# qfall/tools

Measured on AMD Instinct MI355X. Metric: preimages/sec (whole node) + HBM-BW% for samp_p, n=512 q~2^30 batch=4096, higher is better.
Workload: dtype f64+int64

## Files before the change

include/psf_mi355x.h:

```cpp
#ifndef PSF_MI355X_H
#define PSF_MI355X_H
#include <stddef.h>
#include <stdint.h>

#ifdef __cplusplus
extern "C" {
#endif

typedef int psf_status;
enum {
  PSF_OK = 0,
  PSF_ERR_PARAM = 1,
  PSF_ERR_NOT_PD = 2,
  PSF_ERR_DOMAIN = 3,
  PSF_ERR_MODULUS = 4,
  PSF_ERR_NO_SOLUTION = 5,
  PSF_ERR_NO_KEY = 6,
  PSF_ERR_HIP = 7,
  PSF_ERR_UNSUPPORTED = 8,
  PSF_ERR_SAMPLER = 9
};

const char* psf_status_string(psf_status);
psf_status psf_device_info(int device, char* name, size_t name_len, int* compute_units);
// ... 162 lines not shown

psf_status psfp_samp_p_dev(psfp_handle*, uint64_t seed, uint64_t first_index, size_t B,
                           const uint64_t* d_u, int64_t* d_e, void* stream);
psf_status psfp_samp_p_dev_many(psfp_handle*, size_t count, const uint64_t* seeds, const uint64_t* first_indices, size_t B,
                                const uint64_t* d_u, int64_t* d_e, void* stream);
psf_status psfp_samp_d_dev(psfp_handle*, uint64_t seed, uint64_t first_index, size_t B, int64_t* d_e, void* stream);
psf_status psfp_f_a_dev(psfp_handle*, size_t B, const int64_t* d_e, uint64_t* d_u, uint8_t* d_ok, void* stream);
psf_status psfp_last_status(psfp_handle*);
psf_status psfp_uniform_targets_dev(psfp_handle*, uint64_t seed, uint64_t first_index, size_t B, uint64_t* d_u, void* stream);
psf_status psf_narrow_rows_dev(const int64_t* d_src, int32_t* d_dst, size_t count, int* d_overflow, int device, void* stream);

psf_status psfp_samp_p_stages(psfp_handle*, uint64_t seed, uint64_t first_index, size_t B, const uint64_t* u,
                              double* d, double* x, int64_t* p, uint64_t* v, int64_t* z, int64_t* e);
psf_status psfp_enable_timing(psfp_handle*, int on);
psf_status psfp_get_timing(psfp_handle*, char* names, size_t names_len, double* ms, size_t* count);
enum {
  PSFP_PLAN_ONE_LAUNCH = 0,
  PSFP_PLAN_PRODUCT,
  PSFP_PLAN_RT, PSFP_PLAN_NB, PSFP_PLAN_NCG,
  PSFP_PLAN_BC,
  PSFP_PLAN_COMPACT,
  PSFP_PLAN_GR, PSFP_PLAN_GC,
  PSFP_PLAN_TAIL,
  PSFP_PLAN_ROUND,
  PSFP_PLAN_SYN_FORM,
  PSFP_PLAN_SYN_SPLITS, PSFP_PLAN_SYN_FOLD128, PSFP_PLAN_SYN_POW2, PSFP_PLAN_SYN_WAVE_COMBINE,
  PSFP_PLAN_GADGET,
  PSFP_PLAN_K32,
  PSFP_PLAN_GQ_P,
  PSFP_PLAN_RECOMBINE,
  PSFP_PLAN_NBF,
  PSFP_PLAN_RC_BIG,
  PSFP_PLAN_RSPLITS,
  PSFP_PLAN_FIELDS
};
enum { PSFP_PRODUCT_TASKS = 0, PSFP_PRODUCT_TILES64 = 1, PSFP_PRODUCT_TILES32 = 2, PSFP_PRODUCT_TILES96 = 3, PSFP_PRODUCT_BIG = 4 };
enum { PSFP_ROUND_TAB = 0, PSFP_ROUND_TAB_ROW = 1, PSFP_ROUND_LEAN = 2, PSFP_ROUND_WAVE = 3 };
enum { PSFP_ZQ_SMALL = 0, PSFP_ZQ_SMALL32 = 1, PSFP_ZQ_MFMA = 2 };
enum { PSFP_GADGET_WAVE = 0, PSFP_GADGET_ROW = 1, PSFP_GADGET_QUAD = 2, PSFP_GADGET_QUEUE = 3, PSFP_GADGET_LOCKSTEP = 4 };
enum { PSFP_RECOMBINE_SMALL = 0, PSFP_RECOMBINE_SMALL2 = 1, PSFP_RECOMBINE_WG = 2, PSFP_RECOMBINE_TILES = 3 };
psf_status psfp_query_plan(const psfp_handle*, size_t B, int* fields, size_t count);
psf_status psfp_get_last_plan(const psfp_handle*, int* fields, size_t count);

typedef struct psfgpv_handle psfgpv_handle;
typedef struct {
  psf_gadget_params gp;
  double s;
  int32_t device;
  uint32_t flags;
} psfgpv_params;

psf_status psfgpv_create(const psfgpv_params* params, psfgpv_handle** out);
void       psfgpv_destroy(psfgpv_handle*);
size_t     psfgpv_m(const psfgpv_handle*);
psf_status psfgpv_trap_gen(psfgpv_handle*, uint64_t seed);
psf_status psfgpv_load_key(psfgpv_handle*, const uint64_t* A, const int32_t* basis_t, const double* gso_t);
psf_status psfgpv_export_key(const psfgpv_handle*, uint64_t* A, int8_t* R, int32_t* basis_t, double* gso_t);
psf_status psfgpv_samp_d(psfgpv_handle*, uint64_t seed, uint64_t first_index, size_t B, int64_t* e);
psf_status psfgpv_samp_p(psfgpv_handle*, uint64_t seed, uint64_t first_index, size_t B, const uint64_t* u, int64_t* e);
psf_status psfgpv_samp_p_dev(psfgpv_handle*, uint64_t seed, uint64_t first_index, size_t B, const uint64_t* d_u, int64_t* d_e, void* stream);
psf_status psfgpv_samp_p_dev_many(psfgpv_handle*, size_t count, const uint64_t* seeds, const uint64_t* first_indices, size_t B,
                                  const uint64_t* d_u, int64_t* d_e, void* stream);
psf_status psfgpv_samp_p_async(psfgpv_handle*, uint64_t seed, uint64_t first_index, size_t B, const uint64_t* u, int64_t* e);
psf_status psfgpv_wait(psfgpv_handle*);
uint64_t   psfgpv_async_next_ticket(const psfgpv_handle*);
psf_status psfgpv_wait_ticket(psfgpv_handle*, uint64_t ticket);
// ... 48 lines not shown
```

tools_amd/csrc/psfp.hip:

```cpp
#include <hip/hip_runtime.h>
#include <cmath>
#include <cstdio>
#include <cstdlib>
#include <cstring>
#include <chrono>
#include <string>
#include <thread>
#include <atomic>
#include <mutex>
#include <functional>
#include <vector>
#include "psf_hip_util.hpp"
#include "psf_host.hpp"
#include "psf_kernels.hpp"
#include "psf_stream_kernels.hpp"
#include "psf_gpv_kernels.hpp"
#include "psf_np_kernels.hpp"
#include "psf_chol_kernels.hpp"
#include "psf_gemm_kernels.hpp"
#include "psf_hostpipe.hpp"
#include "psf_ntt_api.hpp"

struct KeygenClock {
  bool on; const char* what; std::chrono::steady_clock::time_point t0, last;
  explicit KeygenClock(const char* w) : on(psf_exp_env("PSF_KEYGEN_TIMING") != nullptr), what(w) { if (on) { hipDeviceSynchronize(); t0 = last = std::chrono::steady_clock::now(); } }
  void mark(const char* phase) {
    if (!on) return;
    hipDeviceSynchronize();
    const auto now = std::chrono::steady_clock::now();
    std::fprintf(stderr, "[keygen %s] %-28s %8.2f ms (at %8.2f)\n", what, phase, std::chrono::duration<double, std::milli>(now - last).count(), std::chrono::duration<double, std::milli>(now - t0).count());
    last = now;
  }
};

#define PSFP_FLAG_NO_PERTURB 1u

using namespace psf;

static inline unsigned grid_for(size_t total, unsigned block = 256, unsigned cap = 256 * 16) {
  size_t g = (total + block - 1) / block;
  if (g < 1) g = 1;
  return (unsigned)(g > cap ? cap : g);
}
#define PSFP_QUIESCE(h) do { const psf_status rw__ = psfp_wait(h); if (rw__ != PSF_OK) return rw__; } while (0)

struct TimingSlot { std::string name; Event e0, e1; };

// ... 17 lines not shown
  bool wide;
  bool has_key = false;
  NormBound dom = {{0, 0, 0}};
  bool has_pub = false;
  bool has_R = false;
  DevArr<uint64_t> dA;
  DevArr<int8_t> dR;
  size_t ldr = 0;
  DevArr<double> dLt;
  size_t M_pad = 0, nbi = 0, nkb = 0;
  bool structured = false;
  size_t mL = 0, nbiL = 0;
  DevArr<int8_t> dR8;
  bool r8_valid = false;
  bool r8_pending = false;
  Event evR8; hipStream_t r8_stream = nullptr;
  DevArr<uint32_t> dR2, dA32; DevArr<int> dR2bad; PinArr<int> hR2bad; Event evSmall;
  DevArr<uint32_t> dA32T;
  DevArr<uint64_t> dPartF;
  int small_state = 0;
  double g_const = 0, h_const = 0;
  DevArr<int32_t> dRng;
  DevArr<int32_t> dSk; DevArr<double> dGso, dNorm2; DevArr<SampleZParams> dSz;
  DevArr<uint64_t> dGvec;
  DevArr<int8_t> dA8; int NA = 0; size_t n_pad = 0, K_pad = 0;
  ZqConsts zc;
  std::vector<int64_t> hSk; std::vector<double> hGso;
  SampleZParams szR, szSR;
  DevArr<uint32_t> dSzTab; uint32_t szF = 0;
  size_t ld = 0, mb_pad = 0;
  DevArr<int> dFail;
  int zq_split_cap = 1;
  bool gadget_queue = true;
  HostPipe hp;
  uint32_t normals_ncf = 0;
  hipStream_t last_stream = nullptr;
  Stream side; Event evSide;
  bool timing = false;
  std::vector<TimingSlot> slots;
  double multi_launched_ms = -1.0, multi_done_ms = -1.0;
  int last_plan[PSFP_PLAN_FIELDS] = {0}; bool has_last_plan = false;
};

static void ensure_small_copies(psfp_handle* h, hipStream_t st) {
  if ((h->prm.flags & PSFP_FLAG_NO_PERTURB) || h->small_state >= 2) return;
  if (h->small_state == 1) {
    if (hipEventQuery(h->evSmall) == hipSuccess) h->small_state = *h->hR2bad ? 3 : 2;
    return;
  }
  const size_t ng = h->ldr / 16;
  if (!h->dR2) {
    if (h->dR2.alloc(h->mb * ng) != hipSuccess || h->dR2bad.alloc(1) != hipSuccess ||
        h->hR2bad.alloc(1) != hipSuccess || hipEventCreateWithFlags(h->evSmall.put(), hipEventDisableTiming) != hipSuccess) { h->small_state = 4; return; }
    if (h->q <= (1ull << 32) && h->dA32.alloc(h->n * h->m) != hipSuccess) { h->small_state = 4; return; }
    if (h->q <= (1ull << 32) && h->n % 8 == 0 && h->dA32T.alloc(h->n * h->m) != hipSuccess) (void)hipGetLastError();
  }
  hipMemsetAsync(h->dR2bad, 0, sizeof(int), st);
  hipLaunchKernelGGL(k_pack_R2, dim3(grid_for(h->mb * ng, 256, 256 * 32)), dim3(256), 0, st, h->dR, h->ldr, h->mb, h->dR2, h->dR2bad);
  if (h->dA32) hipLaunchKernelGGL(k_narrow_A32, dim3(grid_for(h->n * h->m, 256, 256 * 32)), dim3(256), 0, st, h->dA, h->n * h->m, h->dA32);
  if (h->dA32T) hipLaunchKernelGGL(k_transpose_A32, dim3((unsigned)((h->m + 31) / 32), (unsigned)((h->n + 31) / 32)), dim3(256), 0, st, h->dA, h->n, h->m, h->dA32T);
  hipMemcpyAsync(h->hR2bad, h->dR2bad, sizeof(int), hipMemcpyDeviceToHost, st);
  hipEventRecord(h->evSmall, st);
  h->small_state = 1;
}

static void ensure_R8(psfp_handle* h, hipStream_t st) {
// ... 291 lines not shown
  const auto gvec = gen_gadget_vec_mod(h->k, gp.base, gp.q);
  HIP_TRY(h->dSk.alloc(sk32.size()));
  HIP_TRY(h->dGso.alloc(h->hGso.size()));
  HIP_TRY(h->dNorm2.alloc(h->k));
  HIP_TRY(h->dSz.alloc(h->k));
  HIP_TRY(h->dGvec.alloc(h->k));
  HIP_TRY(hipMemcpy(h->dSk, sk32.data(), sk32.size() * sizeof(int32_t), hipMemcpyHostToDevice));
  HIP_TRY(hipMemcpy(h->dGso, h->hGso.data(), h->hGso.size() * sizeof(double), hipMemcpyHostToDevice));
  HIP_TRY(hipMemcpy(h->dNorm2, norm2.data(), h->k * sizeof(double), hipMemcpyHostToDevice));
  HIP_TRY(hipMemcpy(h->dSz, sz.data(), h->k * sizeof(SampleZParams), hipMemcpyHostToDevice));
  HIP_TRY(hipMemcpy(h->dGvec, gvec.data(), h->k * sizeof(uint64_t), hipMemcpyHostToDevice));
  HIP_TRY(hipFuncSetAttribute(reinterpret_cast<const void*>(k_recombine_mfma), hipFuncAttributeMaxDynamicSharedMemorySize, RC_LDS));
  HIP_TRY(hipFuncSetAttribute(reinterpret_cast<const void*>(k_recombine_mfma_big), hipFuncAttributeMaxDynamicSharedMemorySize, RCB_LDS));
  HIP_TRY(hipFuncSetAttribute(reinterpret_cast<const void*>(k_recombine_small<1>), hipFuncAttributeMaxDynamicSharedMemorySize, 150 * 1024));
  HIP_TRY(hipFuncSetAttribute(reinterpret_cast<const void*>(k_recombine_small<2>), hipFuncAttributeMaxDynamicSharedMemorySize, 150 * 1024));
  HIP_TRY(hipFuncSetAttribute(reinterpret_cast<const void*>(k_recombine_small<4>), hipFuncAttributeMaxDynamicSharedMemorySize, 150 * 1024));
  HIP_TRY(hipFuncSetAttribute(reinterpret_cast<const void*>(k_recombine_small2<1>), hipFuncAttributeMaxDynamicSharedMemorySize, 150 * 1024));
  HIP_TRY(hipFuncSetAttribute(reinterpret_cast<const void*>(k_recombine_small2<2>), hipFuncAttributeMaxDynamicSharedMemorySize, 150 * 1024));
  HIP_TRY(hipFuncSetAttribute(reinterpret_cast<const void*>(k_recombine_small2<4>), hipFuncAttributeMaxDynamicSharedMemorySize, 150 * 1024));
  HIP_TRY(hipFuncSetAttribute(reinterpret_cast<const void*>(k_rd2_mfma), hipFuncAttributeMaxDynamicSharedMemorySize, 3 * (1 + kFixPlanes) * 4096));
  HIP_TRY(hipFuncSetAttribute(reinterpret_cast<const void*>(k_gadget), hipFuncAttributeMaxDynamicSharedMemorySize, (int)gadget_lds_bytes(h->k)));
  HIP_TRY(hipFuncSetAttribute(reinterpret_cast<const void*>(k_recombine_wg<1, 4>), hipFuncAttributeMaxDynamicSharedMemorySize, (int)RW_LDS));
  HIP_TRY(hipFuncSetAttribute(reinterpret_cast<const void*>(k_recombine_wg<2, 8>), hipFuncAttributeMaxDynamicSharedMemorySize, (int)RW_LDS));
  HIP_TRY(hipFuncSetAttribute(reinterpret_cast<const void*>(k_recombine_wg<3, 8>), hipFuncAttributeMaxDynamicSharedMemorySize, (int)RW_LDS));
  HIP_TRY(hipFuncSetAttribute(reinterpret_cast<const void*>(k_recombine_wg<4, 8>), hipFuncAttributeMaxDynamicSharedMemorySize, (int)RW_LDS));
  HIP_TRY(hipFuncSetAttribute(reinterpret_cast<const void*>(k_trmm_stream_wg32<TSW_H, TSW_NBUF, 0>), hipFuncAttributeMaxDynamicSharedMemorySize, (int)TSW32_LDS));
  HIP_TRY(hipFuncSetAttribute(reinterpret_cast<const void*>(k_trmm_stream_wg32<TSW_H, TSW_NBUF, 1>), hipFuncAttributeMaxDynamicSharedMemorySize, (int)TSW32_LDS));
  HIP_TRY(hipFuncSetAttribute(reinterpret_cast<const void*>(k_trmm_stream_wg<TSW64_H, TSW64_NBUF, 0, 2>), hipFuncAttributeMaxDynamicSharedMemorySize, (int)TSW_LDS));
  HIP_TRY(hipFuncSetAttribute(reinterpret_cast<const void*>(k_trmm_stream_wg<TSW64_H, TSW64_NBUF, 1, 2>), hipFuncAttributeMaxDynamicSharedMemorySize, (int)TSW_LDS));
  HIP_TRY(hipFuncSetAttribute(reinterpret_cast<const void*>(k_gadget_queue<true>), hipFuncAttributeMaxDynamicSharedMemorySize, (int)gadget_queue_lds_bytes(h->k)));
  HIP_TRY(hipFuncSetAttribute(reinterpret_cast<const void*>(k_gadget_queue<false>), hipFuncAttributeMaxDynamicSharedMemorySize, (int)gadget_queue_lds_bytes(h->k)));
  if (const char* env = psf_exp_env("PSF_GADGET_QUEUE")) h->gadget_queue = std::atoi(env) != 0;
  for (int64_t v : h->hSk) if (v > 32767 || v < -32768) h->gadget_queue = false;
  return PSF_OK;
}

static void hp_prewarm(psfp_handle* h) {
  if (h->m < 8192) return;
  if (const char* env = psf_exp_env("PSF_HOST_PREWARM")) if (std::atoi(env) == 0) return;
  if (h->hp.hp_warm.joinable()) h->hp.hp_warm.join();
  try {
    h->hp.hp_warm = std::thread([h]() { if (hipSetDevice(h->prm.device) == hipSuccess) (void)hp_ensure(h->hp, h->prm.device, 0, 0, 0, true); });
  } catch (...) { }
}
void psfp_destroy(psfp_handle* h) {
  if (!h) return;
  hipSetDevice(h->prm.device);
  delete h;
}

size_t psfp_m(const psfp_handle* h) { return h ? h->m : 0; }

static void launch_chol_diag(hipStream_t st, double* P, size_t ld, size_t off, int nb, double* dLi, int* dinfo, size_t report_base) {
  hipLaunchKernelGGL(k_chol_diag_inv, dim3(1), dim3(256), CH_DIAG_LDS, st, P, ld, off, nb, dLi, dinfo, report_base);
}
static bool prepare_chol_diag() {
  return hipFuncSetAttribute(reinterpret_cast<const void*>(k_chol_diag_inv), hipFuncAttributeMaxDynamicSharedMemorySize, (int)CH_DIAG_LDS) == hipSuccess;
}

static psf_status build_sqrt_sigma2_stream(psfp_handle* h, double nf_r2, double s2, double b2p1, const double* d_sig, const double* dS_dense = nullptr) {
  const size_t m = h->mL;
  const int nbi = (int)h->nbiL;
  const int nP = (nbi + 1) / 2;
  const size_t PW = 2 * TR_BM;
  const size_t prow = (size_t)nbi * TR_BM;
  auto splits_for = [](int wgs, int units) {
// ... 410 lines not shown
  } else {
    const dim3 grid((unsigned)z.splits, (unsigned)((h->n + 15) / 16));
    if (z.form == ZqPlan::SMALL32)
      hipLaunchKernelGGL(by_cols(ncols, k_syndrome_small32<1>, k_syndrome_small32<2>, k_syndrome_small32<4>), grid, dim3(512), 0, st, h->dA32, h->n, h->m, P, ld, ncols, h->q, 16,
                         h->dPart, h->n_pad, (size_t)0);
    else
      hipLaunchKernelGGL(by_cols(ncols, k_syndrome_small<1>, k_syndrome_small<2>, k_syndrome_small<4>), grid, dim3(512), 0, st, h->dA, h->n, h->m, P, ld, ncols, h->q, 16,
                         h->dPart, h->n_pad, (size_t)0);
  }
  hipLaunchKernelGGL(z.wave_combine ? k_zq_combine_wave<false> : k_zq_combine, dim3(z.wave_combine ? (unsigned)((h->n * ncols + 3) / 4) : grid_for(h->n * ncols, 256, 256 * 32)),
                     dim3(256), 0, st, mode, h->dPart, z.splits, h->n, h->n_pad, ld, ncols, h->q, U, out, ldo, (size_t)0);
}

struct SampCall {
  bool keep_fail = false;
  bool whole_batch = false;
  const HostStage* before_u = nullptr;
  const std::chrono::steady_clock::time_point* launched = nullptr;
};

struct SampPlan {
  size_t nbj = 0;
  bool one_launch = false;
  int bc = 0; uint32_t ncf = 0, nseg = 0; size_t nwaves = 0;
  enum Product : uint8_t { TASKS, TILES64, TILES32, TILES96, BIG } product = BIG;
  int RT = 2, NB = 1, ncg = 1;
  bool compact = false; int GR = 8, GC = 4;
  bool tail = false; int tail_ntask = 0, tail_rt = 2;
  enum Round : uint8_t { ROUND_TAB, ROUND_TAB_ROW, ROUND_LEAN, ROUND_WAVE } round = ROUND_WAVE;
  uint32_t seg = 0; size_t rwaves = 0;
  ZqPlan syn;
  enum Gadget : uint8_t { G_WAVE, G_ROW, G_QUAD, G_QUEUE, G_LOCKSTEP } gadget = G_LOCKSTEP;
  bool k32 = false; int gq_p = 0;
  enum Recombine : uint8_t { R_SMALL, R_SMALL2, R_WG, R_TILES } recombine = R_TILES;
  size_t rc_lds = 0; unsigned rc_wgs = 0; int nbf = 0;
  bool rc_big = false; int rsplits = 1, kps = 0;
  bool small_copies = false, r8 = false;
};

struct BatchDims { size_t nbj; int zq_split_cap; };

static SampPlan plan_samp_p(const psfp_handle* h, size_t B, const SampCall& call, const BatchDims* bd = nullptr) {
  SampPlan p;
  const size_t m = h->m;
  const size_t nbj = p.nbj = bd ? bd->nbj : round_up(B, TR_BN) / TR_BN;
  size_t fused_max = 64;
  if (const char* e = psf_exp_env("PSF_FUSED_MAX")) fused_max = (size_t)std::atol(e);
  p.one_launch = !h->structured && !call.whole_batch && h->gadget_queue && m <= (size_t)FS_MAX_M && h->n <= 64 && B <= fused_max;
  if (p.one_launch) return p;
  bool stream = B <= 1472 || (B >= 1537 && B <= 1728) || (h->mL < 16384 && B <= 2048);
  if (const char* e = psf_exp_env("PSF_TRMM_STREAM_MAX")) stream = B <= std::min<size_t>((size_t)std::atol(e), 2048);
  const char* shape = psf_exp_env("PSF_TRMM_STREAM_SHAPE");
  p.NB = B <= 16 ? 1 : B <= 64 ? 2 : 4;
  size_t wg_min = 33;
  if (const char* e = psf_exp_env("PSF_STREAM_WG")) wg_min = std::atol(e) > 0 ? (size_t)std::atol(e) : (size_t)-1;
  size_t wg_max = 64;
  if (const char* e = psf_exp_env("PSF_STREAM_WG_MAX")) wg_max = std::min<size_t>((size_t)std::atol(e), 64);
  const bool small_factor = h->mL < 16384;
  bool wg192 = stream && ((B > 128 && B <= 960 && (((B + 63) / 64) & 1) != 0) || B > 1088 || (small_factor && B > 64)) && !shape;
  if (const char* e = psf_exp_env("PSF_STREAM_WG192")) {
    long lo = 0, hi = 0;
    wg192 = std::sscanf(e, "%ld:%ld", &lo, &hi) == 2 && lo >= 65 && hi <= 2048 && stream && B >= (size_t)lo && B <= (size_t)hi && !shape;
  }
  const bool wg = stream && ((B >= wg_min && B <= wg_max) || wg192) && !shape;
  const char* e32 = psf_exp_env("PSF_STREAM_WG32");
  const bool wg32 = stream && !wg && B >= 17 && B <= 32 && !shape && !(e32 && std::atoi(e32) == 0);
// ... 25 lines not shown
      if (const char* e = psf_exp_env("PSF_FUSED_RT")) p.tail_rt = std::atoi(e) == 1 ? 1 : 2;
      p.tail_ntask = ((int)((h->mL + 15) / 16) + p.tail_rt - 1) / p.tail_rt;
      p.tail = true;
    }
  }
  p.r8 = h->structured;
  const char* renv = psf_exp_env("PSF_ROUND");
  if (h->szR.sh == 16 && !(renv && !std::strcmp(renv, "wave"))) {
    p.seg = prl_segment(m * B);
    if (const char* e = psf_exp_env("PSF_PRL_SEG")) { const long v = std::atol(e); if (v >= 64 && v <= PRL_SEG && v % 64 == 0) p.seg = (uint32_t)v; }
    p.round = SampPlan::ROUND_LEAN;
    if (h->szF && !(renv && !std::strcmp(renv, "lean"))) {
      if (B % 64 == 0 && B >= 1024 && B <= (size_t)PRL_SEG && (size_t)p.seg > B) p.seg = (uint32_t)B;
      p.round = (size_t)p.seg == B ? SampPlan::ROUND_TAB_ROW : SampPlan::ROUND_TAB;
    }
    p.rwaves = (m * B + p.seg - 1) / p.seg;
  } else p.rwaves = (m * B + PR_SEG - 1) / PR_SEG;
  p.syn = plan_zq(h, B, true, bd ? bd->zq_split_cap : -1);
  p.small_copies |= p.syn.form != ZqPlan::MFMA;
  const size_t nB = h->n * B;
  const char* genv = psf_exp_env("PSF_GADGET_WAVE");
  const size_t wave_max = genv ? (size_t)std::atol(genv) : 2048;
  const char* genvq = psf_exp_env("PSF_GADGET_QUAD");
  const size_t quad_max = genvq ? (size_t)std::atol(genvq) : 98304;
  const char* genvr = psf_exp_env("PSF_GADGET_ROW");
  const size_t row_max = genvr ? (size_t)std::atol(genvr) : 10240;
  p.k32 = h->k <= 32;
  if (!h->gadget_queue) p.gadget = SampPlan::G_LOCKSTEP;
  else if (nB <= wave_max) p.gadget = SampPlan::G_WAVE;
  else if (nB <= row_max && h->k <= 64) p.gadget = SampPlan::G_ROW;
  else if (nB <= quad_max && h->k <= 64) p.gadget = SampPlan::G_QUAD;
  else {
    p.gadget = SampPlan::G_QUEUE;
    p.gq_p = gq_problems_for((uint32_t)h->k, nB);
    if (const char* e = psf_exp_env("PSF_GQ_P")) { const int v = std::atoi(e); if (v >= 1 && v <= 128 && (v & (v - 1)) == 0) p.gq_p = v; }
  }
  size_t small_max = 4;
  if (const char* e = psf_exp_env("PSF_RECOMBINE_SMALL")) small_max = std::min<size_t>((size_t)std::atol(e), 4);
  p.rc_lds = 32 * (h->ldr / 16) * B;
  size_t rs_max = 448;
  if (const char* e = psf_exp_env("PSF_RECOMBINE_STREAM")) rs_max = (size_t)std::min<long>(std::atol(e), 1024);
  if (B <= small_max && p.rc_lds <= 150 * 1024) {
    p.recombine = h->small_state == 2 ? SampPlan::R_SMALL2 : SampPlan::R_SMALL;
    p.rc_wgs = (unsigned)std::min<size_t>((h->mb + 7) / 8, p.rc_lds > 64 * 1024 ? 256 : 512);
    p.small_copies = true;
  } else if (B <= rs_max && h->ldr % 128 == 0 && h->mb >= 64) {
    p.recombine = SampPlan::R_WG;
    p.nbf = B > 64 ? 4 : (int)((B + 15) / 16);
  } else {
    p.recombine = SampPlan::R_TILES;
    p.rc_big = (B % 256 == 0 || B > rs_max) && h->mb >= 512 && (h->ldr / 64) % 2 == 0;
    p.r8 = p.r8 || p.rc_big;
    const unsigned tiles = (unsigned)((B + 127) / 128) * (unsigned)((h->mb + 127) / 128);
    const int nks = (int)(h->ldr / 64);
    p.kps = nks;
    if (!p.rc_big && tiles < 1024 && nks >= 16) {
      const int splits = (int)(2048 / tiles);
      p.kps = std::max((nks + splits - 1) / splits, 8);
      p.kps += p.kps & 1;
      p.rsplits = (nks + p.kps - 1) / p.kps;
    }
  }
  return p;
}

static_assert(SampPlan::BIG == PSFP_PRODUCT_BIG && SampPlan::TILES96 == PSFP_PRODUCT_TILES96 && SampPlan::TILES64 == PSFP_PRODUCT_TILES64 && SampPlan::ROUND_WAVE == PSFP_ROUND_WAVE &&
              SampPlan::ROUND_TAB_ROW == PSFP_ROUND_TAB_ROW && ZqPlan::MFMA == PSFP_ZQ_MFMA && ZqPlan::SMALL32 == PSFP_ZQ_SMALL32 && SampPlan::G_LOCKSTEP == PSFP_GADGET_LOCKSTEP &&
              SampPlan::G_QUAD == PSFP_GADGET_QUAD && SampPlan::R_TILES == PSFP_RECOMBINE_TILES && SampPlan::R_SMALL2 == PSFP_RECOMBINE_SMALL2 && PSFP_PLAN_RSPLITS == 22,
              "the enumerators of include/psf_mi355x.h follow SampPlan");
static void plan_fields(const SampPlan& p, int* f) {
  const int v[PSFP_PLAN_FIELDS] = {p.one_launch, p.product, p.RT, p.NB, p.ncg, p.bc, p.compact, p.GR, p.GC, p.tail, p.round, p.syn.form, p.syn.splits, p.syn.fold128, p.syn.pow2,
                                   p.syn.wave_combine, p.gadget, p.k32, p.gq_p, p.recombine, p.nbf, p.rc_big, p.rsplits};
  std::memcpy(f, v, sizeof(v));
}

static void prepare_samp_p(psfp_handle* h, hipStream_t st, SampPlan& p) {
  if (p.small_copies) ensure_small_copies(h, st);
  if (p.tail) {
    const size_t need = (size_t)p.tail_ntask * h->n * 2;
    if (h->dPartF.grow(need) != hipSuccess) (void)hipGetLastError();
    p.tail = h->dPartF != nullptr;
  }
  if (p.r8) ensure_R8(h, st);
}

static void normals_stage(psfp_handle* h, hipStream_t st, const SampPlan& p, uint64_t seed, uint64_t first_index, size_t B) {
  ScopedTimer t(h, st, "k_normals");
  const NormalsFixed fx = h->structured ? NormalsFixed{h->mb, h->dD8, h->ldr * h->ld, h->ld, h->dX, h->h_const} : NormalsFixed{0, nullptr, 0, 0, nullptr, 0.0};
  hipLaunchKernelGGL(k_normals_wave, dim3((unsigned)((p.nwaves + 3) / 4)), dim3(256), 0, st, seed, first_index, h->m, B, h->nkb, p.nbj, h->dDt, h->dFail, fx, p.ncf, p.nseg);
}

static void product_stage(psfp_handle* h, hipStream_t st, const SampPlan& p, size_t B) {
  ScopedTimer t(h, st, "k_trmm_f64");
  const size_t row_hi = h->structured ? h->mb : h->M_pad;
  if (p.product == SampPlan::BIG) {
    hipLaunchKernelGGL(k_trmm_f64_big, dim3(tr_grid_size(((int)h->nbiL + 1) / 2, (int)p.nbj, p.GR, p.GC)), dim3(256), 0, st, h->dLt, h->dDt, h->dX, (int)h->nbiL, (int)p.nbj,
                       h->nkb, h->ld, p.GR, p.GC, row_hi);
    return;
  }
  auto geom = [&](int rt, int ncg, int bc) { StreamGeom g; g.ntile = ((int)((h->mL + 15) / 16) + rt - 1) / rt; g.ncg = ncg; g.ntask = g.ntile * ncg; g.bc = bc; return g; };
  auto go = [&](auto kern, const StreamGeom& g, unsigned grid, unsigned block, size_t lds) { hipLaunchKernelGGL(kern, dim3(grid), dim3(block), lds, st, h->dLt, h->dDt, h->dX, g, h->nkb, h->ld, row_hi); };
  auto cd = [&](auto k0, auto k1) { return p.compact ? k1 : k0; };
  const auto wg64 = cd(k_trmm_stream_wg<TSW64_H, TSW64_NBUF, 0, 2>, k_trmm_stream_wg<TSW64_H, TSW64_NBUF, 1, 2>);
  const auto wg32 = cd(k_trmm_stream_wg32<TSW_H, TSW_NBUF, 0>, k_trmm_stream_wg32<TSW_H, TSW_NBUF, 1>);
  StreamGeom g = geom(4, p.product == SampPlan::TILES96 ? 1 : p.ncg, 0);
// ... 40 lines not shown
    case SampPlan::ROUND_TAB:
    case SampPlan::ROUND_TAB_ROW:
      hipLaunchKernelGGL(p.round == SampPlan::ROUND_TAB_ROW ? k_perturb_round_tab<true> : k_perturb_round_tab<false>, grid, dim3(256), (size_t)h->szR.n_int * h->szF * sizeof(uint32_t),
                         st, seed, first_index, m, B, ld, h->dX, h->szR, h->dP, h->dFail, p.seg, SzTable{h->dSzTab, h->szF, h->szR.n_int});
      break;
    case SampPlan::ROUND_LEAN:
      hipLaunchKernelGGL(k_perturb_round_lean, grid, dim3(256), 0, st, seed, first_index, m, B, ld, h->dX, h->szR, h->dP, h->dFail, p.seg);
      break;
    case SampPlan::ROUND_WAVE:
      hipLaunchKernelGGL(k_perturb_round_wave, grid, dim3(256), 0, st, seed, first_index, m, B, ld, h->dX, h->szR, h->dP, h->dFail);
      break;
  }
}

static void syndrome_stage(psfp_handle* h, hipStream_t st, const SampPlan& p, size_t B, const uint64_t* d_u) {
  ScopedTimer t(h, st, "k_zq_matmul(syndrome)");
  if (p.tail)
    hipLaunchKernelGGL((k_zq_combine_wave<true>), dim3((unsigned)((h->n * B + 3) / 4)), dim3(256), 0, st, ZQ_SYNDROME, h->dPartF, p.tail_ntask, h->n, h->n, (size_t)p.bc, B, h->q, d_u, h->dV, h->ld, (size_t)0);
  else launch_zq(h, st, p.syn, ZQ_SYNDROME, h->dP, h->dP8, B, d_u, h->dV, h->ld);
}

static void gadget_stage(psfp_handle* h, hipStream_t st, const SampPlan& p, uint64_t seed, uint64_t first_index, size_t B) {
  const size_t ld = h->ld, nB = h->n * B;
  ScopedTimer t(h, st, "k_gadget");
  const GadgetTablesQ tq{h->dSk, h->dGso, h->dNorm2, h->dSz, h->dRng};
  auto go = [&](auto kern, dim3 grid, size_t lds, auto tables, auto... extra) {
    hipLaunchKernelGGL(kern, grid, dim3(256), lds, st, seed, first_index, (uint32_t)h->n, (uint32_t)h->k, h->q, h->prm.gp.base, B, ld, h->dV, tables, h->dZlo, h->dZhi, h->dFail, extra...);
  };
  switch (p.gadget) {
    case SampPlan::G_WAVE: go(k_gadget_wave, dim3((unsigned)((nB + 3) / 4)), 0, tq); break;
    case SampPlan::G_ROW: go(p.k32 ? k_gadget_quad<2, 16> : k_gadget_quad<4, 16>, dim3((unsigned)((nB + 15) / 16)), 0, tq); break;
    case SampPlan::G_QUAD: go(p.k32 ? k_gadget_quad<8> : k_gadget_quad<16>, dim3((unsigned)((nB + 63) / 64)), 0, tq); break;
    case SampPlan::G_QUEUE:
      go(p.gq_p == 128 ? k_gadget_queue<true> : k_gadget_queue<false>, dim3((unsigned)((nB + (size_t)GQ_WAVES * p.gq_p - 1) / ((size_t)GQ_WAVES * p.gq_p))),
         gadget_queue_lds_bytes(h->k, p.gq_p), tq, p.gq_p);
      break;
    case SampPlan::G_LOCKSTEP:
      go(k_gadget, dim3((unsigned)((B + 255) / 256), (unsigned)h->n), gadget_lds_bytes(h->k), GadgetTables{h->dSk, h->dGso, h->dNorm2, h->dSz});
      break;
  }
}

static void recombine_stage(psfp_handle* h, hipStream_t st, const SampPlan& p, size_t B, int64_t* d_e) {
  const size_t ld = h->ld, m = h->m;
  ScopedTimer t(h, st, "k_recombine");
  auto bottom = [&](size_t cols, int zero_top) {
    hipLaunchKernelGGL(k_recombine_bottom, dim3((unsigned)((B + 63) / 64), (unsigned)((cols + 63) / 64)), dim3(256), 0, st, h->mb, h->w, h->dZlo, h->dZhi, ld, h->dP, B, d_e, m, zero_top);
  };
  switch (p.recombine) {
    case SampPlan::R_SMALL2:
      hipLaunchKernelGGL(by_cols(B, k_recombine_small2<1>, k_recombine_small2<2>, k_recombine_small2<4>), dim3(p.rc_wgs), dim3(512), p.rc_lds, st, h->dR2, h->ldr, h->mb, h->w,
                         h->dZlo, h->dZhi, ld, h->dP, B, d_e, m);
      break;
    case SampPlan::R_SMALL:
      hipLaunchKernelGGL(by_cols(B, k_recombine_small<1>, k_recombine_small<2>, k_recombine_small<4>), dim3(p.rc_wgs), dim3(512), p.rc_lds, st, h->dR, h->ldr, h->mb, h->w,
                         h->dZlo, h->dZhi, ld, h->dP, B, d_e, m);
      break;
    case SampPlan::R_WG: {
      bottom(h->w, 0);
      hipLaunchKernelGGL((p.nbf == 1 ? k_recombine_wg<1, 4> : p.nbf == 2 ? k_recombine_wg<2, 8> : p.nbf == 3 ? k_recombine_wg<3, 8> : k_recombine_wg<4, 8>),
                         dim3((unsigned)((h->mb + 63) / 64), (unsigned)((B + 63) / 64)), dim3(64 * (p.nbf == 1 ? 4 : 8)), RW_LDS, st, h->dR, h->ldr, h->mb, (int)(h->ldr / 128),
                         h->dZlo, h->dZhi, ld, h->dFail, h->dP, B, d_e, m);
      break;
    }
    case SampPlan::R_TILES:
      if (p.rc_big) {
// ... 401 lines not shown
```

tools_amd/psf.py:

```python
import ctypes as C

import numpy as np

from . import _ffi
from ._ffi import GadgetParams, GpvParams, PsfpParams, RingParams, PsfError, _p, check, lib


def _many(fn, h, d_u_ptr, d_e_ptr, B, seeds, first_indices, stream):
    s = np.ascontiguousarray(np.asarray(seeds, dtype=np.uint64).reshape(-1))
    f = np.ascontiguousarray(np.asarray(first_indices, dtype=np.uint64).reshape(-1))
    if s.shape != f.shape:
        raise PsfError(_ffi.ERR_PARAM, "samp_p_dev_many")
    check(fn(h, C.c_size_t(s.size), _p(s, C.c_uint64), _p(f, C.c_uint64), C.c_size_t(B), C.c_void_p(d_u_ptr), C.c_void_p(d_e_ptr),
             C.c_void_p(stream or 0)), "samp_p_dev_many")


class GadgetParameters:

    def __init__(self, n, k, m_bar, base, q):
        self.c = GadgetParams(n, k, m_bar, base, q)

    @classmethod
    def init_default(cls, n, q):
        c = GadgetParams()
# ... 191 lines not shown
        check(lib().psfp_f_a_dev(self._h, C.c_size_t(B), C.c_void_p(d_e_ptr), C.c_void_p(d_u_ptr), C.c_void_p(d_ok_ptr),
                                 C.c_void_p(stream or 0)), "f_a_dev")

    def uniform_targets_dev(self, d_u_ptr, B, seed=0, first_index=0, stream=None):
        check(lib().psfp_uniform_targets_dev(self._h, C.c_uint64(seed), C.c_uint64(first_index), C.c_size_t(B),
                                             C.c_void_p(d_u_ptr), C.c_void_p(stream or 0)), "uniform_targets_dev")

    def last_status(self):
        return lib().psfp_last_status(self._h)

    def query_plan(self, B):
        f = (C.c_int * len(PLAN_FIELDS))()
        check(lib().psfp_query_plan(self._h, C.c_size_t(B), f, C.c_size_t(len(PLAN_FIELDS))), "query_plan")
        return _plan_dict(f)

    def last_plan(self):
        f = (C.c_int * len(PLAN_FIELDS))()
        check(lib().psfp_get_last_plan(self._h, f, C.c_size_t(len(PLAN_FIELDS))), "last_plan")
        return _plan_dict(f)

    def enable_timing(self, on=True):
        check(lib().psfp_enable_timing(self._h, C.c_int(1 if on else 0)), "enable_timing")

    def get_timing(self):
        names = C.create_string_buffer(4096)
        ms = (C.c_double * 64)()
        cnt = C.c_size_t(64)
        check(lib().psfp_get_timing(self._h, names, C.c_size_t(4096), ms, C.byref(cnt)), "get_timing")
        nm = names.value.decode().split(";") if names.value else []
        return list(zip(nm, list(ms)[:cnt.value]))


PLAN_FIELDS = ("one_launch", "product", "RT", "NB", "ncg", "bc", "compact", "GR", "GC", "tail", "round", "syn.form", "syn.splits", "syn.fold128", "syn.pow2",
               "syn.wave_combine", "gadget", "k32", "gq_p", "recombine", "nbf", "rc_big", "rsplits")
PLAN_ENUMS = {
    "product": ("TASKS", "TILES64", "TILES32", "TILES96", "BIG"),
    "round": ("ROUND_TAB", "ROUND_TAB_ROW", "ROUND_LEAN", "ROUND_WAVE"),
    "syn.form": ("SMALL", "SMALL32", "MFMA"),
    "gadget": ("G_WAVE", "G_ROW", "G_QUAD", "G_QUEUE", "G_LOCKSTEP"),
    "recombine": ("R_SMALL", "R_SMALL2", "R_WG", "R_TILES"),
}


def _plan_dict(fields):
    return {name: PLAN_ENUMS[name][v] if name in PLAN_ENUMS else int(v) for name, v in zip(PLAN_FIELDS, fields)}


def samp_p_multi(psfs, u, seed=0, first_index=0, out=None):
    n, m = psfs[0].n, psfs[0].m
    u2 = np.ascontiguousarray(u, dtype=np.uint64).reshape(-1, n)
    B = u2.shape[0]
    e = np.zeros((B, m), dtype=np.int64) if out is None else out
    assert e.dtype == np.int64 and e.shape == (B, m) and e.flags["C_CONTIGUOUS"]
    arr = (C.c_void_p * len(psfs))(*[p._h for p in psfs])
    check(lib().psfp_samp_p_multi(arr, C.c_int(len(psfs)), C.c_uint64(seed), C.c_uint64(first_index), C.c_size_t(B), _p(u2, C.c_uint64), _p(e, C.c_int64)),
          "samp_p_multi")
    return e


def multi_timing(psf):
    a, b = C.c_double(0), C.c_double(0)
    check(lib().psfp_get_multi_timing(psf._h, C.byref(a), C.byref(b)), "multi_timing")
    return a.value, b.value


class PSFGPV:

# ... 301 lines not shown
```

Before: 70040.

## Add persistent lane-per-problem gadget sampler with producer/consumer ring

Adds a new k_gadget_lane kernel for the gadget-queue path. Each lane owns one gadget problem. A persistent grid sized to CUs pulls 64-problem chunks through an atomic counter, precomputes GSO dot products into an LDS ring, and runs the per-step discrete Gaussian sampling with deferred writes. The kernel is enabled when the gadget basis is bidiagonal and the digits fit in 64 bits. It is meant to remove the per-problem workgroup organisation and load imbalance of k_gadget_queue, at the cost of high register pressure (a 32-double xr array) and added control-flow complexity.

New measurement: 70660, median of 6. Within noise of the previous version (+0.9%).

```diff
diff --git a/include/psf_mi355x.h b/include/psf_mi355x.h
--- a/include/psf_mi355x.h
+++ b/include/psf_mi355x.h
@@ -218,6 +218,7 @@
   PSFP_PLAN_NBF,
   PSFP_PLAN_RC_BIG,
   PSFP_PLAN_RSPLITS,
+  PSFP_PLAN_GQ_LANE,
   PSFP_PLAN_FIELDS
 };
 enum { PSFP_PRODUCT_TASKS = 0, PSFP_PRODUCT_TILES64 = 1, PSFP_PRODUCT_TILES32 = 2, PSFP_PRODUCT_TILES96 = 3, PSFP_PRODUCT_BIG = 4 };
diff --git a/tools_amd/csrc/psf_gadget_kernels.hpp b/tools_amd/csrc/psf_gadget_kernels.hpp
--- /dev/null
+++ b/tools_amd/csrc/psf_gadget_kernels.hpp
@@ -0,0 +1,214 @@
+#pragma once
+#include "psf_kernels.hpp"
+
+namespace psf {
+
+constexpr int GL_WAVES = 4;
+constexpr int GL_RING = 16;
+constexpr int GL_SLOTS = 2;
+constexpr int GL_KMAX = 32;
+constexpr int GL_WG_PER_CU = 3;
+#ifndef PSF_GL_GROUPS
+#define PSF_GL_GROUPS 3
+#endif
+constexpr int GL_GROUPS = PSF_GL_GROUPS;
+
+struct GlStep { double norm2, gsub; SampleZParams sz; int32_t sd, ss; };
+
+__host__ inline uint32_t gadget_lane_digit_bits(uint64_t base) { uint32_t b = 1; while (b < 63 && (1ull << b) < base) ++b; return b; }
+
+__global__ __launch_bounds__(256) __attribute__((amdgpu_waves_per_eu(3, 3))) void k_gadget_lane(uint64_t seed, uint64_t first_index, uint32_t n, uint32_t k, uint64_t q, uint64_t base, size_t B, size_t ld,
+                                                     const uint64_t* __restrict__ V, GadgetTablesQ tb, int8_t* __restrict__ Zlo, int8_t* __restrict__ Zhi,
+                                                     int* __restrict__ fail, unsigned long long* __restrict__ next_chunk, uint32_t bits) {
+  __shared__ __attribute__((aligned(16))) double s_gT[GL_KMAX * GL_KMAX];
+  __shared__ __attribute__((aligned(16))) GlStep s_step[GL_KMAX];
+  __shared__ double s_pre_all[GL_WAVES][GL_RING * 64];
+  __shared__ uint64_t s_dig_all[GL_WAVES][GL_SLOTS * 64];
+  __shared__ uint2 s_jb_all[GL_WAVES][GL_SLOTS * 64];
+  const int tid = threadIdx.x, lane = tid & 63, wave = tid >> 6;
+  const int ki = (int)k;
+  for (int e = tid; e < GL_KMAX * GL_KMAX; e += 256) {
+    const int i = e / GL_KMAX, r = e % GL_KMAX;
+    s_gT[e] = (i < ki && r <= i) ? tb.gso[(size_t)r * k + i] : 0.0;
+  }
+  for (int i = tid; i < ki; i += 256) {
+    GlStep g;
+    g.norm2 = tb.norm2[i];
+    g.gsub = i + 1 < ki ? tb.gso[(size_t)(i + 1) * k + i] : 0.0;
+    g.sz = tb.sz[i];
+    g.sd = tb.Sk[(size_t)i * k + i];
+    g.ss = i + 1 < ki ? tb.Sk[(size_t)(i + 1) * k + i] : 0;
+    s_step[i] = g;
+  }
+  __syncthreads();
+  double* s_pre = s_pre_all[wave];
+  uint64_t* s_dig = s_dig_all[wave];
+  uint2* s_jb = s_jb_all[wave];
+
+  const size_t total = (size_t)n * B;
+  const uint32_t B32 = (uint32_t)B;
+  const uint64_t dmask = (1ull << bits) - 1;
+  const bool q_pow2 = (q & (q - 1)) == 0, base_pow2 = (base & (base - 1)) == 0;
+  int f = 0, anyhi = 0;
+
+  int pc = 0, pi = ki - 1, s_prod = 0;
+  bool prod_done = false;
+  double xr[GL_KMAX];
+#pragma unroll
+  for (int r = 0; r < GL_KMAX; ++r) xr[r] = 0.0;
+
+  int mycoh = 0, step = -1, s = 0;
+  bool has = false;
+  uint64_t dig = 0;
+  int w = 0, msd = 0, mss = 0;
+  uint32_t myj = 0, myb = 0, t = 0;
+  double cen = 0.0, inv_s = 0.0;
+  SzRange rg{0, 1, 0, 16};
+  uint32_t idx_lo = 0, tw = 0, coord = 0;
+  float c_rel = 0.f, inv_s_f = 0.f;
+  bool narrow = false;
+
+  bool pend = false;
+  int pend_val = 0;
+  size_t pend_addr = 0;
+  auto emit = [&](size_t addr, int val) {
+    const int32_t zz = -val;
+    const int32_t zl = (int32_t)(int8_t)(zz & 0xff);
+    const int32_t zh = (zz - zl) >> 8;
+    Zlo[addr] = (int8_t)zl;
+    Zhi[addr] = (int8_t)zh;
+    if (zh) anyhi = 1;
+  };
+
+  for (;;) {
+    if (!prod_done) {
+      const int adopted = mycoh - (step < 0 ? 1 : 0);
+      const bool lag = s_prod - s >= GL_RING || (pi == ki - 1 && adopted + GL_SLOTS <= pc);
+      if (__ballot(lag) == 0) {
+        if (pi == ki - 1) {
+          unsigned long long c0 = 0;
+          if (lane == 0) c0 = atomicAdd(next_chunk, 1ull);
+          const uint32_t c0l = __builtin_amdgcn_readfirstlane((uint32_t)c0), c0h = __builtin_amdgcn_readfirstlane((uint32_t)(c0 >> 32));
+          const size_t pid0 = (((size_t)c0h << 32) | c0l) * 64;
+          if (pid0 >= total) prod_done = true;
+          else {
+            const uint32_t j0 = (uint32_t)(pid0 / B), o = (uint32_t)(pid0 % B) + (uint32_t)lane;
+            uint32_t j, b;
+            if (B32 >= 64u) { const bool wrap = o >= B32; j = j0 + (wrap ? 1u : 0u); b = wrap ? o - B32 : o; }
+            else { j = j0 + o / B32; b = o % B32; }
+            const bool valid = pid0 + (size_t)lane < total;
+            uint64_t v = valid ? V[(size_t)j * ld + b] : 0;
+            v = q_pow2 ? (v & (q - 1)) : v % q;
+            uint64_t dg = v;
+            if (!base_pow2) {
+              dg = 0;
+              for (int r = 0; r < ki; ++r) { const uint64_t d = v % base; v = (v - d) / base; dg |= d << (r * (int)bits); }
+            }
+#pragma unroll
+            for (int r = 0; r < GL_KMAX; ++r) xr[r] = r < ki ? (double)(-(int)((dg >> ((r < ki ? r : 0) * (int)bits)) & dmask)) : 0.0;
+            const int slot = (pc & (GL_SLOTS - 1)) * 64 + lane;
+            s_dig[slot] = dg;
+            s_jb[slot] = make_uint2(valid ? j : 0xffffffffu, b);
+          }
+        }
+        if (!prod_done) {
+          const double* g = s_gT + pi * GL_KMAX;
+          double dot = 0.0;
+#pragma unroll
+          for (int blk = 0; blk < GL_KMAX / 8; ++blk)
+            if (blk * 8 <= pi) {
+#pragma unroll
+              for (int r = blk * 8; r < blk * 8 + 8; ++r) dot = fma(xr[r], g[r], dot);
+            }
+          s_pre[(s_prod & (GL_RING - 1)) * 64 + lane] = dot;
+          ++s_prod;
+          if (--pi < 0) { pi = ki - 1; ++pc; }
+        }
+      }
+    }
+    if (!has && s_prod - s > 0) {
+      if (step < 0) {
+        const int slot = (mycoh & (GL_SLOTS - 1)) * 64 + lane;
+        const uint2 jb = s_jb[slot];
+        if (jb.x == 0xffffffffu) { ++mycoh; s += ki; }
+        else {
+          dig = s_dig[slot];
+          myj = jb.x; myb = jb.y;
+          step = ki - 1;
+          w = 0;
+          const uint64_t index = first_index + myb;
+          idx_lo = (uint32_t)index;
+          tw = tag_word(TAG_GADGET, index);
+        }
+      }
+      if (step >= 0) {
+        const GlStep g = s_step[step];
+        const double pre = s_pre[(s & (GL_RING - 1)) * 64 + lane];
+        cen = fma((double)w, g.gsub, pre) / g.norm2;
+        const SampleZParams sp = g.sz;
+        msd = g.sd; mss = g.ss;
+        inv_s = sp.inv_s;
+        coord = myj * k + (uint32_t)step;
+        narrow = sp.sh == 16 && fabs(cen) < 0x1.0p30;
+        if (narrow) {
+          const double cc = ceil(cen);
+          const bool integral = cc == cen;
+          rg.lo = (long long)((int)cc - (int)sp.c6);
+          rg.N = integral ? sp.n_int : sp.n_int - 1;
+          rg.thr = integral ? sp.thr_int : sp.thr_frac;
+          rg.sh = 16;
+          c_rel = (float)((double)rg.lo - cen);
+          inv_s_f = (float)sp.inv_s;
+        } else rg = sz_range(cen, sp);
+        t = 0;
+        has = true;
+      }
+    }
+    bool accept = false;
+    long long x = 0;
+    if (has) {
+#pragma clang loop unroll(disable)
+      for (int g = 0; g < GL_GROUPS && !accept; ++g) {
+        accept = narrow ? sz_group4_narrow(seed, coord, idx_lo, tw, t, rg, cen, inv_s, c_rel, inv_s_f, &x)
+                        : sz_group4(seed, coord, idx_lo, tw, t, rg, cen, inv_s, &x);
+        if (!accept && ++t >= kMaxAttempts / 4) { accept = true; f = 1; x = (long long)floor(cen + 0.5); }
+      }
+    }
+    if (accept) {
+      if (x > 16000 || x < -16000) f = 1;
+      const int z = (int)x;
+      const int nv0 = -(int)((dig >> (step * (int)bits)) & dmask) - z * msd;
+      if (nv0 > 32767 || nv0 < -32768) f = 1;
+      bool wr = pend;
+      int val = pend_val;
+      size_t addr = pend_addr;
+      uint32_t c15 = 0;
+      if (step + 1 < ki) {
+        const int nv1 = w - z * mss;
+        if (nv1 > 32767 || nv1 < -32768) f = 1;
+        val = (int)(int16_t)nv1;
+        const uint32_t c = coord + 1;
+        c15 = c & 15;
+        addr = ((size_t)(c >> 4) * ld + myb) * 16 + c15;
+        wr = true;
+      } else pend = false;
+      if (wr) emit(addr, val);
+      w = (int)(int16_t)nv0;
+      if (step == 0) {
+        pend = true;
+        pend_val = w;
+        pend_addr = c15 ? addr - 1 : addr - (16 * ld - 15);
+        ++mycoh;
+      }
+      --step;
+      ++s;
+      has = false;
+    }
+    if (prod_done && __ballot(has || s_prod - s > 0) == 0) break;
+  }
+  if (pend) emit(pend_addr, pend_val);
+  if (f) atomicOr(fail, 1);
+  if (anyhi) atomicOr(fail + 1, 1);
+}
+
+}
diff --git a/tools_amd/csrc/psfp.hip b/tools_amd/csrc/psfp.hip
--- a/tools_amd/csrc/psfp.hip
+++ b/tools_amd/csrc/psfp.hip
@@ -13,6 +13,7 @@
 #include "psf_hip_util.hpp"
 #include "psf_host.hpp"
 #include "psf_kernels.hpp"
+#include "psf_gadget_kernels.hpp"
 #include "psf_stream_kernels.hpp"
 #include "psf_gpv_kernels.hpp"
 #include "psf_np_kernels.hpp"
@@ -96,6 +97,10 @@
   DevArr<int> dFail;
   int zq_split_cap = 1;
   bool gadget_queue = true;
+  bool gq_lane = false;
+  uint32_t gq_bits = 0;
+  DevArr<unsigned long long> dGqNext;
+  int cus = 0;
   HostPipe hp;
   uint32_t normals_ncf = 0;
   hipStream_t last_stream = nullptr;
@@ -453,6 +458,16 @@
   HIP_TRY(hipFuncSetAttribute(reinterpret_cast<const void*>(k_gadget_queue<false>), hipFuncAttributeMaxDynamicSharedMemorySize, (int)gadget_queue_lds_bytes(h->k)));
   if (const char* env = psf_exp_env("PSF_GADGET_QUEUE")) h->gadget_queue = std::atoi(env) != 0;
   for (int64_t v : h->hSk) if (v > 32767 || v < -32768) h->gadget_queue = false;
+  h->gq_bits = gadget_lane_digit_bits(gp.base);
+  h->gq_lane = h->gadget_queue && h->k >= 2 && h->k <= (size_t)GL_KMAX && gp.base >= 2 && gp.base <= 32767 && h->k * h->gq_bits <= 64;
+  for (size_t col = 0; col < h->k && h->gq_lane; ++col)
+    for (size_t r = 0; r < h->k; ++r) {
+      if (r != col && r != col + 1 && h->hSk[r * h->k + col] != 0) h->gq_lane = false;
+      if (r > col + 1 && h->hGso[r * h->k + col] != 0.0) h->gq_lane = false;
+    }
+  if (const char* env = psf_exp_env("PSF_GQ_LANE")) if (std::atoi(env) == 0) h->gq_lane = false;
+  if (h->gq_lane) HIP_TRY(h->dGqNext.alloc(1));
+  HIP_TRY(hipDeviceGetAttribute(&h->cus, hipDeviceAttributeMultiprocessorCount, prm->device));
   return PSF_OK;
 }
 
@@ -929,6 +944,7 @@
   ZqPlan syn;
   enum Gadget : uint8_t { G_WAVE, G_ROW, G_QUAD, G_QUEUE, G_LOCKSTEP } gadget = G_LOCKSTEP;
   bool k32 = false; int gq_p = 0;
+  bool gq_lane = false;
   enum Recombine : uint8_t { R_SMALL, R_SMALL2, R_WG, R_TILES } recombine = R_TILES;
   size_t rc_lds = 0; unsigned rc_wgs = 0; int nbf = 0;
   bool rc_big = false; int rsplits = 1, kps = 0;
@@ -1020,8 +1036,11 @@
   else if (nB <= quad_max && h->k <= 64) p.gadget = SampPlan::G_QUAD;
   else {
     p.gadget = SampPlan::G_QUEUE;
-    p.gq_p = gq_problems_for((uint32_t)h->k, nB);
-    if (const char* e = psf_exp_env("PSF_GQ_P")) { const int v = std::atoi(e); if (v >= 1 && v <= 128 && (v & (v - 1)) == 0) p.gq_p = v; }
+    p.gq_lane = h->gq_lane && B < (1ull << 32);
+    if (!p.gq_lane) {
+      p.gq_p = gq_problems_for((uint32_t)h->k, nB);
+      if (const char* e = psf_exp_env("PSF_GQ_P")) { const int v = std::atoi(e); if (v >= 1 && v <= 128 && (v & (v - 1)) == 0) p.gq_p = v; }
+    }
   }
   size_t small_max = 4;
   if (const char* e = psf_exp_env("PSF_RECOMBINE_SMALL")) small_max = std::min<size_t>((size_t)std::atol(e), 4);
@@ -1054,11 +1073,12 @@
 
 static_assert(SampPlan::BIG == PSFP_PRODUCT_BIG && SampPlan::TILES96 == PSFP_PRODUCT_TILES96 && SampPlan::TILES64 == PSFP_PRODUCT_TILES64 && SampPlan::ROUND_WAVE == PSFP_ROUND_WAVE &&
               SampPlan::ROUND_TAB_ROW == PSFP_ROUND_TAB_ROW && ZqPlan::MFMA == PSFP_ZQ_MFMA && ZqPlan::SMALL32 == PSFP_ZQ_SMALL32 && SampPlan::G_LOCKSTEP == PSFP_GADGET_LOCKSTEP &&
-              SampPlan::G_QUAD == PSFP_GADGET_QUAD && SampPlan::R_TILES == PSFP_RECOMBINE_TILES && SampPlan::R_SMALL2 == PSFP_RECOMBINE_SMALL2 && PSFP_PLAN_RSPLITS == 22,
+              SampPlan::G_QUAD == PSFP_GADGET_QUAD && SampPlan::R_TILES == PSFP_RECOMBINE_TILES && SampPlan::R_SMALL2 == PSFP_RECOMBINE_SMALL2 && PSFP_PLAN_RSPLITS == 22 &&
+              PSFP_PLAN_GQ_LANE == 23,
               "the enumerators of include/psf_mi355x.h follow SampPlan");
 static void plan_fields(const SampPlan& p, int* f) {
   const int v[PSFP_PLAN_FIELDS] = {p.one_launch, p.product, p.RT, p.NB, p.ncg, p.bc, p.compact, p.GR, p.GC, p.tail, p.round, p.syn.form, p.syn.splits, p.syn.fold128, p.syn.pow2,
-                                   p.syn.wave_combine, p.gadget, p.k32, p.gq_p, p.recombine, p.nbf, p.rc_big, p.rsplits};
+                                   p.syn.wave_combine, p.gadget, p.k32, p.gq_p, p.recombine, p.nbf, p.rc_big, p.rsplits, p.gq_lane};
   std::memcpy(f, v, sizeof(v));
 }
 
@@ -1165,6 +1185,13 @@
     case SampPlan::G_ROW: go(p.k32 ? k_gadget_quad<2, 16> : k_gadget_quad<4, 16>, dim3((unsigned)((nB + 15) / 16)), 0, tq); break;
     case SampPlan::G_QUAD: go(p.k32 ? k_gadget_quad<8> : k_gadget_quad<16>, dim3((unsigned)((nB + 63) / 64)), 0, tq); break;
     case SampPlan::G_QUEUE:
+      if (p.gq_lane) {
+        const size_t chunks = (nB + 63) / 64;
+        hipMemsetAsync(h->dGqNext, 0, sizeof(unsigned long long), st);
+        go(k_gadget_lane, dim3((unsigned)std::min<size_t>((chunks + GL_WAVES - 1) / GL_WAVES, (size_t)GL_WG_PER_CU * (size_t)std::max(h->cus, 1))), 0, tq,
+           (unsigned long long*)h->dGqNext, h->gq_bits);
+        break;
+      }
       go(p.gq_p == 128 ? k_gadget_queue<true> : k_gadget_queue<false>, dim3((unsigned)((nB + (size_t)GQ_WAVES * p.gq_p - 1) / ((size_t)GQ_WAVES * p.gq_p))),
          gadget_queue_lds_bytes(h->k, p.gq_p), tq, p.gq_p);
       break;
diff --git a/tools_amd/psf.py b/tools_amd/psf.py
--- a/tools_amd/psf.py
+++ b/tools_amd/psf.py
@@ -247,7 +247,7 @@
 
 
 PLAN_FIELDS = ("one_launch", "product", "RT", "NB", "ncg", "bc", "compact", "GR", "GC", "tail", "round", "syn.form", "syn.splits", "syn.fold128", "syn.pow2",
-               "syn.wave_combine", "gadget", "k32", "gq_p", "recombine", "nbf", "rc_big", "rsplits")
+               "syn.wave_combine", "gadget", "k32", "gq_p", "recombine", "nbf", "rc_big", "rsplits", "gq_lane")
 PLAN_ENUMS = {
     "product": ("TASKS", "TILES64", "TILES32", "TILES96", "BIG"),
     "round": ("ROUND_TAB", "ROUND_TAB_ROW", "ROUND_LEAN", "ROUND_WAVE"),
```
